# SchusterLab/quantum-optimal-control

Hardware: AMD Instinct MI355X
Metric: GRAPE iterations/sec (fwd+bwd+Adam) at n=32 k=4 steps=500 (higher is better)
Workload: dtype f64; 1 GPU; C2 3-transmon-size unitary gate: n=32 k=4 steps=500 m=8 Taylor(T,s)=(5,3), 64 independent control seeds per GPU (aggregate over seeds), reg_coeffs={}; seeds_per_gpu=64, total_seeds=64, chunks=16, stream_groups=1, ranks_seen=1, fidelities_gathered=64, devices_distinct=1, transport=single process, transport_fallback=False

## Files before the change

quantum-optimal-control_amd/csrc/qoc_mfma_downup.h:

```cpp
#pragma once
#include "qoc_mfma_frag.h"

template <int MQ, int KC, int QA = 8>
__global__ void __launch_bounds__(512) k_mfma_downup(QocDev d, QocMfma mf) {
    constexpr int NT = 2, LDP = F2_LDP, ISZ = 4 * MQ * LDP, VSZ = NT * MQ * 64;
    extern __shared__ __attribute__((aligned(16))) char smem[];
    const int lane = threadIdx.x & 63;
    const int wv = __builtin_amdgcn_readfirstlane(threadIdx.x >> 6);
    const int role = wv & 1, pr = wv >> 1;
    cplx* Hl = (cplx*)smem;
    cplx* img = Hl + (size_t)KC * QFR + (size_t)wv * ISZ;
    cplx* xch = Hl + (size_t)KC * QFR + (size_t)8 * ISZ + (size_t)pr * 2 * VSZ;
    double* gred = (double*)(Hl + (size_t)KC * QFR + (size_t)8 * ISZ + (size_t)4 * 2 * VSZ) + wv * 4 * KC;
    volatile int* flag = (volatile int*)((double*)(Hl + (size_t)KC * QFR + (size_t)8 * ISZ + (size_t)4 * 2 * VSZ) + 8 * 4 * KC) + pr * 2;
    for (int o = threadIdx.x; o < KC * QFR; o += blockDim.x) Hl[o] = o < d.k * QFR ? mf.HfD[QFR + o] : cmake(0.0, 0.0);
    if (lane == 0) flag[role] = 0;
    __syncthreads();
    const int item = blockIdx.x * 4 + pr;
#ifndef QOC_DOWNUP_STAGGER
#define QOC_DOWNUP_STAGGER 2
#endif
    constexpr int STG = QOC_DOWNUP_STAGGER == 4 ? 1 : (QOC_DOWNUP_STAGGER == 2 ? 2 : 0);
    if (item >= d.B * mf.C) { if (STG && lane == 0) flag[role] = 1; return; }
    const int c = item / d.B, b = item - c * d.B;
    if (d.skip_done && d.done[b]) { if (STG && lane == 0) flag[role] = 1; return; }
    if (STG && pr >= STG) {
        volatile int* prev = flag - 2 * STG;
        while (prev[0] == 0 || prev[1] == 0) __builtin_amdgcn_s_sleep(8);
        asm volatile("" ::: "memory");
    }
    const int t0 = c * mf.L, t1 = min(t0 + mf.L, d.steps), tm = t0 + (t1 - t0 + 1) / 2;
    const int lk = lane >> 4, lc = lane & 15, li4 = lane & 3;
    struct Frag { cplx f[NT][8]; };
    struct Vec { cplx v[NT][MQ]; };
    auto product = [&](const Frag& fr, const double sg, double (&re)[NT][MQ], double (&im)[NT][MQ]) {
#pragma unroll
        for (int I = 0; I < NT; ++I)
#pragma unroll
            for (int jb = 0; jb < MQ; ++jb) img[(4 * jb + lk) * LDP + 16 * I + lc] = cmake(re[I][jb], im[I][jb]);
        wave_lds_fence();
        double a[NT][MQ], bq[NT][MQ], cq[NT][MQ];
#pragma unroll
        for (int I = 0; I < NT; ++I)
#pragma unroll
            for (int jb = 0; jb < MQ; ++jb) { a[I][jb] = 0.0; bq[I][jb] = 0.0; cq[I][jb] = 0.0; }
#pragma unroll
        for (int kb = 0; kb < QA; ++kb) {
            cplx v[MQ];
#pragma unroll
            for (int jb = 0; jb < MQ; ++jb) v[jb] = img[(4 * jb + li4) * LDP + 4 * kb + lk];
#pragma unroll
            for (int I = 0; I < NT; ++I) {
                const double br = fr.f[I][kb].x, bi = fr.f[I][kb].y, bs = br + sg * bi;
#pragma unroll
                for (int jb = 0; jb < MQ; ++jb) {
                    a[I][jb] = __builtin_amdgcn_mfma_f64_4x4x4f64(v[jb].x, br, a[I][jb], 0, 0, 0);
                    bq[I][jb] = __builtin_amdgcn_mfma_f64_4x4x4f64(v[jb].y, bi, bq[I][jb], 0, 0, 0);
                    cq[I][jb] = __builtin_amdgcn_mfma_f64_4x4x4f64(v[jb].x + v[jb].y, bs, cq[I][jb], 0, 0, 0);
                }
            }
        }
        asm volatile("" ::: "memory");
#pragma unroll
        for (int I = 0; I < NT; ++I)
#pragma unroll
            for (int jb = 0; jb < MQ; ++jb) {
                re[I][jb] = a[I][jb] - sg * bq[I][jb]; im[I][jb] = cq[I][jb] - a[I][jb] - sg * bq[I][jb];
            }
    };
    auto load_fwd = [&](Frag& fr, int t) {
        const cplx* __restrict__ F = mf.KfD + kitem(mf, d.steps, b, t);
#pragma unroll
        for (int I = 0; I < NT; ++I)
#pragma unroll
            for (int q = 0; q < QA; ++q) fr.f[I][q] = F[((q >> 2) * QQS + 4 * I + (lc >> 2)) * 64 + 16 * (lc & 3) + 4 * (q & 3) + lk];
    };
    auto load_adj = [&](Frag& fr, int t) {
        const cplx* __restrict__ F = mf.KfD + kitem(mf, d.steps, b, t);
#pragma unroll
        for (int I = 0; I < NT; ++I)
#pragma unroll
            for (int q = 0; q < QA; ++q) fr.f[I][q] = F[(I * QQS + q) * 64 + lane];
    };
    cplx* X = mf.LamL + (size_t)b * d.steps * VSZ + lane;
    auto store_x = [&](int t, const double (&re)[NT][MQ], const double (&im)[NT][MQ]) {
        cplx* o = X + (size_t)t * VSZ;
#pragma unroll
        for (int I = 0; I < NT; ++I)
#pragma unroll
            for (int jb = 0; jb < MQ; ++jb) o[(I * MQ + jb) * 64] = cmake(re[I][jb], im[I][jb]);
    };
    auto load_x = [&](Vec& x, int t) {
        const cplx* o = X + (size_t)t * VSZ;
#pragma unroll
        for (int I = 0; I < NT; ++I)
#pragma unroll
            for (int jb = 0; jb < MQ; ++jb) x.v[I][jb] = o[(I * MQ + jb) * 64];
    };
    auto gradient = [&](int t, auto lr, auto li, auto pr_, auto pi_) {
        double g[KC];
#pragma unroll
        for (int kk = 0; kk < KC; ++kk) g[kk] = 0.0;
#pragma unroll
        for (int I = 0; I < NT; ++I)
#pragma unroll
            for (int Jp = 0; Jp < NT; ++Jp) {
                d4 t1v = {0, 0, 0, 0}, t2v = {0, 0, 0, 0}, t3v = {0, 0, 0, 0};
#pragma unroll
                for (int q = 0; q < MQ; ++q) {
                    t1v = QMFMA(lr(I, q), pr_(Jp, q), t1v);
                    t2v = QMFMA(li(I, q), pi_(Jp, q), t2v);
                    t3v = QMFMA(lr(I, q) - li(I, q), pr_(Jp, q) + pi_(Jp, q), t3v);
                }
                const d4 qr = t1v + t2v, qi = t3v - t1v + t2v;
#pragma unroll
                for (int kk = 0; kk < KC; ++kk) {
                    double acc = 0.0;
#pragma unroll
                    for (int r = 0; r < 4 && 4 * I + r < QA; ++r) {
                        const cplx hv = Hl[(size_t)kk * QFR + (Jp * QQS + 4 * I + r) * 64 + lane];
                        acc = fma(hv.x, qr[r], acc);
                        acc = fma(-hv.y, qi[r], acc);
                    }
                    g[kk] += acc;
                }
            }
#pragma unroll
        for (int kk = 0; kk < KC; ++kk) {
            g[kk] += dpp_xor<1>(g[kk]); g[kk] += dpp_xor<2>(g[kk]); g[kk] += dpp_xor<4>(g[kk]); g[kk] += dpp_xor<8>(g[kk]);
        }
        if (lc == 0) {
#pragma unroll
            for (int kk = 0; kk < KC; ++kk) gred[lk * KC + kk] = g[kk];
        }
        wave_lds_fence();
        if (lane < d.k) d.dLdu[((size_t)b * d.k + lane) * d.steps + t] = (gred[lane] + gred[KC + lane]) + (gred[2 * KC + lane] + gred[3 * KC + lane]);
        asm volatile("" ::: "memory");
    };
    auto publish = [&](int which, const double (&re)[NT][MQ], const double (&im)[NT][MQ]) {
#pragma unroll
        for (int I = 0; I < NT; ++I)
#pragma unroll
            for (int jb = 0; jb < MQ; ++jb) xch[which * VSZ + (I * MQ + jb) * 64 + lane] = cmake(re[I][jb], im[I][jb]);
        wave_lds_fence();
        if (lane == 0) flag[which] = 1;
    };
    auto receive = [&](int which, double (&re)[NT][MQ], double (&im)[NT][MQ]) {
        while (flag[which] == 0) __builtin_amdgcn_s_sleep(4);
        asm volatile("" ::: "memory");
#pragma unroll
        for (int I = 0; I < NT; ++I)
#pragma unroll
            for (int jb = 0; jb < MQ; ++jb) { const cplx v = xch[which * VSZ + (I * MQ + jb) * 64 + lane]; re[I][jb] = v.x; im[I][jb] = v.y; }
        wave_lds_fence();
    };
    const size_t vec0 = ((size_t)b * mf.C + c) * VSZ + lane;
    double sre[NT][MQ], sim[NT][MQ];
    Frag k0, k1;
    if (role == 0) {
        const int n = tm - t0;
#pragma unroll
        for (int I = 0; I < NT; ++I)
#pragma unroll
            for (int jb = 0; jb < MQ; ++jb) { const cplx v = mf.BndF[vec0 + (size_t)(I * MQ + jb) * 64]; sre[I][jb] = v.x; sim[I][jb] = v.y; }
        auto up = [&](const Frag& fr, int s) {
            if (s >= n) return;
            product(fr, 1.0, sre, sim);
            store_x(t0 + s, sre, sim);
        };
        load_fwd(k0, t0); asm volatile("" ::: "memory");
        for (int s = 0; s < n; s += 2) {
            load_fwd(k1, t0 + min(s + 1, n - 1)); asm volatile("" ::: "memory"); up(k0, s);
            load_fwd(k0, t0 + min(s + 2, n - 1)); asm volatile("" ::: "memory"); up(k1, s + 1);
        }
        publish(0, sre, sim);
        asm volatile("s_waitcnt vmcnt(0)" ::: "memory");
        Vec x0, x1;
#pragma unroll
        for (int I = 0; I < NT; ++I)
#pragma unroll
            for (int jb = 0; jb < MQ; ++jb) x0.v[I][jb] = cmake(sre[I][jb], sim[I][jb]);
        load_adj(k0, tm - 1); asm volatile("" ::: "memory");
        receive(1, sre, sim);
        auto down = [&](const Frag& fr, const Vec& x, int i) {
            if (i >= n) return;
            gradient(tm - 1 - i, [&](int I, int q) { return sre[I][q]; }, [&](int I, int q) { return sim[I][q]; },
                     [&](int J, int q) { return x.v[J][q].x; }, [&](int J, int q) { return x.v[J][q].y; });
            if (i + 1 < n) product(fr, -1.0, sre, sim);
        };
        for (int i = 0; i < n; i += 2) {
            load_adj(k1, tm - 1 - min(i + 1, n - 1)); load_x(x1, tm - 1 - min(i + 1, n - 1)); asm volatile("" ::: "memory"); down(k0, x0, i);
            load_adj(k0, tm - 1 - min(i + 2, n - 1)); load_x(x0, tm - 1 - min(i + 2, n - 1)); asm volatile("" ::: "memory"); down(k1, x1, i + 1);
        }
    } else {
        const int n = t1 - tm;
        const int nc = max(n, 1);
        const int tl = t1 - 1;
        load_adj(k0, tl);
        cplx bnd[NT][MQ];
#pragma unroll
        for (int I = 0; I < NT; ++I)
#pragma unroll
            for (int jb = 0; jb < MQ; ++jb) bnd[I][jb] = mf.BndA[vec0 + (size_t)(I * MQ + jb) * 64];
        asm volatile("" ::: "memory");
        {
            double zr = 0.0, zi = 0.0;
            {
                const int nm = d.n * d.m;
                const cplx* fin = d.inter + ((size_t)b * (d.steps + 1) + d.steps) * nm;
                for (int o = lane; o < nm; o += 64) {
                    const cplx f = fin[o], w = d.W[o];
                    zr += f.x * w.x + f.y * w.y;
                    zi += f.y * w.x - f.x * w.y;
                }
#pragma unroll
                for (int off = 32; off > 0; off >>= 1) { zr += __shfl_down(zr, off, 64); zi += __shfl_down(zi, off, 64); }
                zr = __shfl(zr, 0, 64); zi = __shfl(zi, 0, 64);
                if (c == mf.C - 1 && lane == 0) {
                    d.zfin[b] = cmake(zr, zi);
                    d.loss[b] = 1.0 - (zr * zr + zi * zi) / ((double)d.m * (double)d.m);
                    d.reg_state[b] = 0.0;
                }
            }
            const cplx z = cmake(zr, zi);
            const double c0 = -2.0 / ((double)d.m * (double)d.m);
#pragma unroll
            for (int I = 0; I < NT; ++I)
#pragma unroll
                for (int jb = 0; jb < MQ; ++jb) {
                    const cplx v = cscale(cmul(z, bnd[I][jb]), c0);
                    sre[I][jb] = v.x; sim[I][jb] = v.y;
                }
        }
        auto down = [&](const Frag& fr, int i) {
            if (i >= n) return;
            store_x(t1 - 1 - i, sre, sim);
            product(fr, -1.0, sre, sim);
        };
        for (int i = 0; i < n; i += 2) {
            load_adj(k1, tl - min(i + 1, nc - 1)); asm volatile("" ::: "memory"); down(k0, i);
            load_adj(k0, tl - min(i + 2, nc - 1)); asm volatile("" ::: "memory"); down(k1, i + 1);
        }
        publish(1, sre, sim);
        asm volatile("s_waitcnt vmcnt(0)" ::: "memory");
        Vec x0, x1;
        const int tf = min(tm, tl);
        load_fwd(k0, tf); load_x(x0, tf); asm volatile("" ::: "memory");
        receive(0, sre, sim);
        auto up = [&](const Frag& fr, const Vec& x, int s) {
            if (s >= n) return;
            product(fr, 1.0, sre, sim);
            gradient(tm + s, [&](int I, int q) { return x.v[I][q].x; }, [&](int I, int q) { return x.v[I][q].y; },
                     [&](int J, int q) { return sre[J][q]; }, [&](int J, int q) { return sim[J][q]; });
        };
        for (int s = 0; s < n; s += 2) {
            load_fwd(k1, tf + min(s + 1, nc - 1)); load_x(x1, tf + min(s + 1, nc - 1)); asm volatile("" ::: "memory"); up(k0, x0, s);
            load_fwd(k0, tf + min(s + 2, nc - 1)); load_x(x0, tf + min(s + 2, nc - 1)); asm volatile("" ::: "memory"); up(k1, x1, s + 1);
        }
    }
}
```

Measured before the change: 60960 GRAPE iterations/s.

## Compute gradient via 4x4x4 f64 MFMA over LDS image blocks instead of d4 QMFMA

Adds a new default gradient path. The left state is written to the wave's LDS image and reloaded as 4x4 blocks, then contracted with 4x4x4 f64 MFMAs one block-row at a time, with block loads interleaved between MFMAs. In the down phase the image written for the gradient is reused by the following multiply, saving one LDS image write per step. The old QMFMA path stays behind QOC_DOWNUP_Q16. The cost is an extra LDS round-trip in the up phase and more MFMA and LDS instructions per gradient.

```diff
diff --git a/quantum-optimal-control_amd/csrc/qoc_mfma_downup.h b/quantum-optimal-control_amd/csrc/qoc_mfma_downup.h
--- a/quantum-optimal-control_amd/csrc/qoc_mfma_downup.h
+++ b/quantum-optimal-control_amd/csrc/qoc_mfma_downup.h
@@ -21,6 +21,10 @@
 #define QOC_DOWNUP_STAGGER 2
 #endif
     constexpr int STG = QOC_DOWNUP_STAGGER == 4 ? 1 : (QOC_DOWNUP_STAGGER == 2 ? 2 : 0);
+#ifndef QOC_DOWNUP_Q16
+#define QOC_DOWNUP_Q16 0
+#endif
+    constexpr bool Q16 = QOC_DOWNUP_Q16 != 0;
     if (item >= d.B * mf.C) { if (STG && lane == 0) flag[role] = 1; return; }
     const int c = item / d.B, b = item - c * d.B;
     if (d.skip_done && d.done[b]) { if (STG && lane == 0) flag[role] = 1; return; }
@@ -33,12 +37,14 @@
     const int lk = lane >> 4, lc = lane & 15, li4 = lane & 3;
     struct Frag { cplx f[NT][8]; };
     struct Vec { cplx v[NT][MQ]; };
-    auto product = [&](const Frag& fr, const double sg, double (&re)[NT][MQ], double (&im)[NT][MQ]) {
-#pragma unroll
-        for (int I = 0; I < NT; ++I)
-#pragma unroll
-            for (int jb = 0; jb < MQ; ++jb) img[(4 * jb + lk) * LDP + 16 * I + lc] = cmake(re[I][jb], im[I][jb]);
+    auto put_image = [&](auto re, auto im) {
+#pragma unroll
+        for (int I = 0; I < NT; ++I)
+#pragma unroll
+            for (int jb = 0; jb < MQ; ++jb) img[(4 * jb + lk) * LDP + 16 * I + lc] = cmake(re(I, jb), im(I, jb));
         wave_lds_fence();
+    };
+    auto multiply = [&](const Frag& fr, const double sg, double (&re)[NT][MQ], double (&im)[NT][MQ]) {
         double a[NT][MQ], bq[NT][MQ], cq[NT][MQ];
 #pragma unroll
         for (int I = 0; I < NT; ++I)
@@ -68,6 +74,10 @@
                 re[I][jb] = a[I][jb] - sg * bq[I][jb]; im[I][jb] = cq[I][jb] - a[I][jb] - sg * bq[I][jb];
             }
     };
+    auto product = [&](const Frag& fr, const double sg, double (&re)[NT][MQ], double (&im)[NT][MQ]) {
+        put_image([&](int I, int jb) { return re[I][jb]; }, [&](int I, int jb) { return im[I][jb]; });
+        multiply(fr, sg, re, im);
+    };
     auto load_fwd = [&](Frag& fr, int t) {
         const cplx* __restrict__ F = mf.KfD + kitem(mf, d.steps, b, t);
 #pragma unroll
@@ -101,30 +111,78 @@
         double g[KC];
 #pragma unroll
         for (int kk = 0; kk < KC; ++kk) g[kk] = 0.0;
-#pragma unroll
-        for (int I = 0; I < NT; ++I)
-#pragma unroll
-            for (int Jp = 0; Jp < NT; ++Jp) {
-                d4 t1v = {0, 0, 0, 0}, t2v = {0, 0, 0, 0}, t3v = {0, 0, 0, 0};
-#pragma unroll
-                for (int q = 0; q < MQ; ++q) {
-                    t1v = QMFMA(lr(I, q), pr_(Jp, q), t1v);
-                    t2v = QMFMA(li(I, q), pi_(Jp, q), t2v);
-                    t3v = QMFMA(lr(I, q) - li(I, q), pr_(Jp, q) + pi_(Jp, q), t3v);
-                }
-                const d4 qr = t1v + t2v, qi = t3v - t1v + t2v;
-#pragma unroll
-                for (int kk = 0; kk < KC; ++kk) {
-                    double acc = 0.0;
-#pragma unroll
-                    for (int r = 0; r < 4 && 4 * I + r < QA; ++r) {
-                        const cplx hv = Hl[(size_t)kk * QFR + (Jp * QQS + 4 * I + r) * 64 + lane];
-                        acc = fma(hv.x, qr[r], acc);
-                        acc = fma(-hv.y, qi[r], acc);
+        if constexpr (Q16) {
+#pragma unroll
+            for (int I = 0; I < NT; ++I)
+#pragma unroll
+                for (int Jp = 0; Jp < NT; ++Jp) {
+                    d4 t1v = {0, 0, 0, 0}, t2v = {0, 0, 0, 0}, t3v = {0, 0, 0, 0};
+#pragma unroll
+                    for (int q = 0; q < MQ; ++q) {
+                        t1v = QMFMA(lr(I, q), pr_(Jp, q), t1v);
+                        t2v = QMFMA(li(I, q), pi_(Jp, q), t2v);
+                        t3v = QMFMA(lr(I, q) - li(I, q), pr_(Jp, q) + pi_(Jp, q), t3v);
                     }
-                    g[kk] += acc;
-                }
-            }
+                    const d4 qr = t1v + t2v, qi = t3v - t1v + t2v;
+#pragma unroll
+                    for (int kk = 0; kk < KC; ++kk) {
+                        double acc = 0.0;
+#pragma unroll
+                        for (int r = 0; r < 4 && 4 * I + r < QA; ++r) {
+                            const cplx hv = Hl[(size_t)kk * QFR + (Jp * QQS + 4 * I + r) * 64 + lane];
+                            acc = fma(hv.x, qr[r], acc);
+                            acc = fma(-hv.y, qi[r], acc);
+                        }
+                        g[kk] += acc;
+                    }
+                }
+        } else {
+            constexpr int RA = KC == 5 ? 1 : 2;
+            cplx bl[RA][MQ];
+            auto blocks = [&](int p) {
+#pragma unroll
+                for (int q = 0; q < MQ; ++q) bl[p % RA][q] = img[(4 * q + lk) * LDP + 4 * p + li4];
+            };
+#pragma unroll
+            for (int p = 0; p < RA; ++p) blocks(p);
+            asm volatile("" ::: "memory");
+            double ps[NT][MQ];
+#pragma unroll
+            for (int Jp = 0; Jp < NT; ++Jp)
+#pragma unroll
+                for (int q = 0; q < MQ; ++q) ps[Jp][q] = pr_(Jp, q) + pi_(Jp, q);
+            double acc[NT][KC];
+#pragma unroll
+            for (int p = 0; p < QA; ++p) {
+                double l1[MQ], l2[MQ], l3[MQ];
+#pragma unroll
+                for (int q = 0; q < MQ; ++q) { l1[q] = bl[p % RA][q].x; l2[q] = bl[p % RA][q].y; l3[q] = l1[q] - l2[q]; }
+#pragma unroll
+                for (int Jp = 0; Jp < NT; ++Jp) {
+                    double t1 = 0.0, t2 = 0.0, t3 = 0.0;
+#pragma unroll
+                    for (int q = 0; q < MQ; ++q) {
+                        t1 = __builtin_amdgcn_mfma_f64_4x4x4f64(l1[q], pr_(Jp, q), t1, 0, 0, 0);
+                        t2 = __builtin_amdgcn_mfma_f64_4x4x4f64(l2[q], pi_(Jp, q), t2, 0, 0, 0);
+                        t3 = __builtin_amdgcn_mfma_f64_4x4x4f64(l3[q], ps[Jp][q], t3, 0, 0, 0);
+                    }
+                    if (Jp == NT - 1 && p + RA < QA) { blocks(p + RA); asm volatile("" ::: "memory"); }
+                    const double qr = t1 + t2, qi = t3 - t1 + t2;
+#pragma unroll
+                    for (int kk = 0; kk < KC; ++kk) {
+                        const cplx hv = Hl[(size_t)kk * QFR + (Jp * QQS + p) * 64 + lane];
+                        acc[Jp][kk] = fma(hv.x, qr, (p & 3) ? acc[Jp][kk] : 0.0);
+                        acc[Jp][kk] = fma(-hv.y, qi, acc[Jp][kk]);
+                    }
+                }
+                if ((p & 3) == 3 || p == QA - 1) {
+#pragma unroll
+                    for (int Jp = 0; Jp < NT; ++Jp)
+#pragma unroll
+                        for (int kk = 0; kk < KC; ++kk) g[kk] += acc[Jp][kk];
+                }
+            }
+        }
 #pragma unroll
         for (int kk = 0; kk < KC; ++kk) {
             g[kk] += dpp_xor<1>(g[kk]); g[kk] += dpp_xor<2>(g[kk]); g[kk] += dpp_xor<4>(g[kk]); g[kk] += dpp_xor<8>(g[kk]);
@@ -184,9 +242,14 @@
         receive(1, sre, sim);
         auto down = [&](const Frag& fr, const Vec& x, int i) {
             if (i >= n) return;
-            gradient(tm - 1 - i, [&](int I, int q) { return sre[I][q]; }, [&](int I, int q) { return sim[I][q]; },
-                     [&](int J, int q) { return x.v[J][q].x; }, [&](int J, int q) { return x.v[J][q].y; });
-            if (i + 1 < n) product(fr, -1.0, sre, sim);
+            const auto lr = [&](int I, int q) { return sre[I][q]; };
+            const auto li = [&](int I, int q) { return sim[I][q]; };
+            if (!Q16) put_image(lr, li);
+            gradient(tm - 1 - i, lr, li, [&](int J, int q) { return x.v[J][q].x; }, [&](int J, int q) { return x.v[J][q].y; });
+            if (i + 1 < n) {
+                if (Q16) put_image(lr, li);
+                multiply(fr, -1.0, sre, sim);
+            }
         };
         for (int i = 0; i < n; i += 2) {
             load_adj(k1, tm - 1 - min(i + 1, n - 1)); load_x(x1, tm - 1 - min(i + 1, n - 1)); asm volatile("" ::: "memory"); down(k0, x0, i);
@@ -250,8 +313,10 @@
         auto up = [&](const Frag& fr, const Vec& x, int s) {
             if (s >= n) return;
             product(fr, 1.0, sre, sim);
-            gradient(tm + s, [&](int I, int q) { return x.v[I][q].x; }, [&](int I, int q) { return x.v[I][q].y; },
-                     [&](int J, int q) { return sre[J][q]; }, [&](int J, int q) { return sim[J][q]; });
+            const auto lr = [&](int I, int q) { return x.v[I][q].x; };
+            const auto li = [&](int I, int q) { return x.v[I][q].y; };
+            if (!Q16) put_image(lr, li);
+            gradient(tm + s, lr, li, [&](int J, int q) { return sre[J][q]; }, [&](int J, int q) { return sim[J][q]; });
         };
         for (int s = 0; s < n; s += 2) {
             load_fwd(k1, tf + min(s + 1, nc - 1)); load_x(x1, tf + min(s + 1, nc - 1)); asm volatile("" ::: "memory"); up(k0, x0, s);
```

After: 60900 GRAPE iterations/s. Within noise of the previous version (-0.1%).
